# 0215Arthur/Pytorch_News_Recommender

Measured on AMD Instinct MI355X. Metric: users/sec (train step) NRMS MIND-small hist=50 cand=5, higher is better.
Workload: dtype f16 (MFMA inputs and saved activations; fp32 accumulate, softmax, loss, master weights and Adam); 1 GPU; configs[1] shapes: NRMS(nrms_v0) train step, 512 users/GPU, hist=50, cand=5, title_len=30, d=300, h=10, q=200, V=45800, dropout=0.2, Adam(lr=1e-3); users_per_gpu=512, global_batch=512, parallelism=dp1, precision=fp16, resident_batches=32

## Files before the change

### pytorch_news_recommender_amd/csrc/fused16_bwd.h

```cpp
#pragma once
#include "fused16.h"

namespace nrms {

constexpr int B16_RED_QKV = 3 * 10 * 32;
constexpr int B16_RED = B16_RED_QKV + 2 * F16_QP;
constexpr int B16_DQ = 96 * 10;

struct Bwd16Args {
    int n_seq, S, d, h, dk, q;
    int n_groups;
    const _Float16* x16;
    const int* pos;
    const int* n_rows;
    const int64_t* ids;
    const int* order;
    const int* order_cnt;
    int n_cls;
    const _Float16* btiles;
    const float* bqkv32;
    const _Float16* qv16;
    const _Float16* ctx16;
    const _Float16* t16;
    const float* w;
    const _Float16* dout16;
    _Float16* dz16;
    _Float16* dctx16;
    _Float16* dqkv16;
    float* red;
    Dropout drop;
    int v1;
    int dbg;
};

__device__ __forceinline__ f32x16 transpose32(const f32x16& x, const h8 (&idf)[2]) {
    f32x16 z = mfma32h(acc_frag(x, 0), idf[0], zero16());
    return mfma32h(acc_frag(x, 1), idf[1], z);
}

__device__ __forceinline__ float regsum(const f32x16& x) {
    float s0 = 0.f, s1 = 0.f, s2 = 0.f, s3 = 0.f;
#pragma unroll
    for (int g = 0; g < 4; ++g) { s0 += x[4 * g]; s1 += x[4 * g + 1]; s2 += x[4 * g + 2]; s3 += x[4 * g + 3]; }
    return (s0 + s1) + (s2 + s3);
}

__device__ __forceinline__ f32x16 transpose_frags(const h8& x0, const h8& x1, const h8 (&idf)[2]) {
    f32x16 z = mfma32h(x0, idf[0], zero16());
    return mfma32h(x1, idf[1], z);
}

constexpr int DX_BM = 256, DX_BK = 64, DX_THREADS = 512;
constexpr int DX_SLABS = B16_DQ / DX_BK;
constexpr int DX_A_BYTES = DX_BM * DX_BK * 2;
constexpr int DX_B_BYTES = DX_BK * F16_KP * 2;
constexpr int DX_SLOT = DX_A_BYTES + DX_B_BYTES;
static_assert(B16_DQ % DX_BK == 0 && F16_KP == 320, "15 slabs of 64; 10 column tiles of 32");
struct Dx16Args {
    int M;
    const int* m_dev;
    const _Float16* a16;
    const _Float16* xtiles;
    int lda, n_slabs;
    float* c;
    int ldc, d;
    const float* sc;
};


size_t bwd16_fused_lds(bool two_blocks);
int launch_bwd16_pool(const Bwd16Args& a, int n_wg, bool two_blocks, hipStream_t stream);
int launch_dx16(const Dx16Args& g, bool out16, hipStream_t stream);
int launch_dout16(long n_seq, int d, int h, int dk, float fixed_scale, float* sc, const float* dout, _Float16* dout16, hipStream_t stream);
int launch_tn16(int geom, const _Float16* A, int lda, int N, const _Float16* B, int ldb, int K, int M, const int* m_dev,
                float* partial, int splits, const int* nmap, const int* kmap, const float* nscale, int ldw, float* dW,
                hipStream_t stream, const char* name, float* dbias = nullptr, const int* blk_list = nullptr, const int* blk_cnt = nullptr,
                int blk_stride = 0);

}
```

### pytorch_news_recommender_amd/csrc/fused16_bwd.hip

```cpp
#include <stdlib.h>

#include "fused16_bwd.h"

namespace nrms {

template <int SB>
__global__ __launch_bounds__(F16_THREADS, SB == 1 ? 8 / F16_WAVES : 1) void fused_bwd16_pool_kernel(Bwd16Args a) {
    extern __shared__ __attribute__((aligned(16))) char smem[];
    float* red = reinterpret_cast<float*>(smem + 3 * F16_SLOT);
    float* stg_t = red + B16_RED;
    float* stg_h = stg_t + F16_WAVES * SB * 2 * F16_QT * 32;
    const int tid = threadIdx.x, lane = tid & 63;
    const int wave = __builtin_amdgcn_readfirstlane(tid >> 6);
    const int l32 = lane & 31, hh = lane >> 5;
    const int S = a.S;
    constexpr int DP = F16_DP, QP = F16_QP;

    for (int i = tid; i < B16_RED; i += F16_THREADS) red[i] = 0.f;

    h8 idf[2], sel[2];
#pragma unroll
    for (int s = 0; s < 2; ++s)
#pragma unroll
        for (int j = 0; j < 8; ++j) {
// ... 429 lines not shown
                            dk = mfma32h(acc_frag(q, 1), acc_frag(dsn, 1), dk);
                        }
                        const h8 dk0 = acc_frag(dk, 0), dk1 = acc_frag(dk, 1);
                        if (drow[jb] >= 0) {
                            *reinterpret_cast<h8*>(orow + 32) = dk0;
                            *reinterpret_cast<h8*>(orow + 32 + 16) = dk1;
                        }
                        sk += regsum(transpose_frags(dk0, dk1, idf));
                    }
                }
                sk += __shfl_xor(sk, 32, 64);
                if (hh == 0) srow[32] = sk;
                float sq = 0.f;
#pragma unroll
                for (int ib = 0; ib < SB; ++ib) {
                    f32x16 dq = zero16();
#pragma unroll
                    for (int jb = 0; jb < SB; ++jb) {
                        const f32x16 k = transpose_frags(kf[jb][0], kf[jb][1], idf);
                        dq = mfma32h(acc_frag(k, 0), sf[jb][ib][0], dq);
                        dq = mfma32h(acc_frag(k, 1), sf[jb][ib][1], dq);
                    }
                    const h8 dq0 = acc_frag(dq, 0), dq1 = acc_frag(dq, 1);
                    if (drow[ib] >= 0) {
                        _Float16* orow = a.dqkv16 + drow[ib] * (long)B16_DQ + head * 96 + 8 * hh;
                        *reinterpret_cast<h8*>(orow) = dq0;
                        *reinterpret_cast<h8*>(orow + 16) = dq1;
                    }
                    sq += regsum(transpose_frags(dq0, dq1, idf));
                }
                sq += __shfl_xor(sq, 32, 64);
                if (hh == 0) srow[0] = sq;
            }
            __syncthreads();
            if (tid < 96) {
                float sum = 0.f;
#pragma unroll
                for (int w = 0; w < F16_WAVES; ++w) sum += stg[(((head & 1) * F16_WAVES + w) * 3) * 32 + tid];
                red[3 * head * 32 + tid] += sum;
            }
            ++n;
        }
#pragma unroll
        for (int b = 0; b < SB; ++b) {
            if (drow[b] >= 0) {
                for (int head = a.h; head < 10; ++head) {
                    _Float16* orow = a.dqkv16 + drow[b] * (long)B16_DQ + head * 96 + 8 * hh;
#pragma unroll
                    for (int c = 0; c < 96; c += 16) *reinterpret_cast<h8*>(orow + c) = z8;
                }
            }
        }
        __syncthreads();
    }
    __syncthreads();
    float* out = a.red + (long)blockIdx.x * B16_RED;
    for (int i = tid; i < B16_RED; i += F16_THREADS) out[i] = red[i];
}

__device__ __forceinline__ float loss_scale_from_max(unsigned max_bits, float fixed) {
    if (fixed > 0.f) return fixed;
    const int e = (int)((max_bits >> 23) & 0xFF) - 127;
    if (max_bits == 0u || e == 128) return 1.0f;
    int k = 6 - e + (int)fmaxf(fixed, -24.f);
    k = k < -100 ? -100 : (k > 100 ? 100 : k);
    return __uint_as_float((unsigned)(k + 127) << 23);
}

__global__ __launch_bounds__(256) void absmax_kernel(long n, const float* x, unsigned* max_bits) {
    unsigned m = 0u;
    const long tid = (long)blockIdx.x * blockDim.x + threadIdx.x, nth = (long)gridDim.x * blockDim.x;
    if ((reinterpret_cast<uintptr_t>(x) & 15) == 0) {
        const f32x4* x4 = reinterpret_cast<const f32x4*>(x);
        const long n4 = n / 4;
        long i = tid;
        for (; i + 3 * nth < n4; i += 4 * nth) {
            f32x4 v[4];
#pragma unroll
            for (int u = 0; u < 4; ++u) v[u] = x4[i + u * nth];
#pragma unroll
            for (int u = 0; u < 4; ++u)
#pragma unroll
                for (int e = 0; e < 4; ++e) m = max(m, __float_as_uint(v[u][e]) & 0x7FFFFFFFu);
        }
        for (; i < n4; i += nth) {
            const f32x4 v = x4[i];
#pragma unroll
            for (int e = 0; e < 4; ++e) m = max(m, __float_as_uint(v[e]) & 0x7FFFFFFFu);
        }
        for (long i = (n & ~3L) + tid; i < n; i += nth) m = max(m, __float_as_uint(x[i]) & 0x7FFFFFFFu);
    } else {
        for (long i = tid; i < n; i += nth) m = max(m, __float_as_uint(x[i]) & 0x7FFFFFFFu);
    }
#pragma unroll
    for (int o = 32; o > 0; o >>= 1) m = max(m, (unsigned)__shfl_xor((int)m, o, 64));
    __shared__ unsigned wmax[4];
    if ((threadIdx.x & 63) == 0) wmax[threadIdx.x >> 6] = m;
    __syncthreads();
    if (threadIdx.x == 0) {
        m = max(max(wmax[0], wmax[1]), max(wmax[2], wmax[3]));
        if (m != 0u) atomicMax(max_bits, m);
    }
}

__device__ __forceinline__ void dout16_rows(long n_seq, int d, int h, int dk, float scale, float* sc, const float* dout, _Float16* dout16,
                                            int n_blocks) {
    if (blockIdx.x == 0 && threadIdx.x == 0) { sc[0] = scale; sc[1] = 1.0f / scale; }
    const long total = n_seq * F16_DP;
    for (long i = (long)blockIdx.x * blockDim.x + threadIdx.x; i < total; i += (long)n_blocks * blockDim.x) {
        const long r = i / F16_DP;
        const int p = (int)(i - r * F16_DP);
        const int b16 = p >> 4, t = p & 15, hh = t >> 3, jj = t & 7;
        const int fpad = 16 * b16 + 8 * (jj >> 2) + 4 * hh + (jj & 3);
        const int head = fpad >> 5, f = fpad & 31;
        float v = 0.f;
        if (head < h && f < dk) v = dout[r * d + head * dk + f] * scale;
        dout16[i] = (_Float16)v;
    }
}

__global__ __launch_bounds__(256) void dout16_kernel(long n_seq, int d, int h, int dk, float fixed_scale, const unsigned* max_bits,
                                                     float* sc, const float* dout, _Float16* dout16) {
    dout16_rows(n_seq, d, h, dk, loss_scale_from_max(*max_bits, fixed_scale), sc, dout, dout16, (int)gridDim.x);
}

struct Prep16bArgs {
    int d, h, dk, q;
    const float* w_qkv;
    const float* b_qkv;
    const float* w_add;
    const float* q_vec;
    float* bqkv32;
    _Float16* btiles;
    _Float16* xtiles;
    _Float16* qv16;
    unsigned* max_bits;
};

__global__ __launch_bounds__(256) void prep16b_kernel(Prep16bArgs a) {
    if (a.max_bits != nullptr && blockIdx.x == 0 && threadIdx.x == 0) *a.max_bits = 0u;
    const float qscale = 1.0f / sqrtf((float)a.dk);
    constexpr int KP = F16_KP;
    const long n1 = (long)4 * a.h * 32 * KP, n2 = (long)30 * 32 * KP, n3 = F16_QP, n4 = (long)3 * a.h * 32;
    for (long i = (long)blockIdx.x * blockDim.x + threadIdx.x; i < n1 + n2 + n3 + n4; i += (long)gridDim.x * blockDim.x) {
        if (i < n1) {
            const int c = (int)(i % KP);
            const long r = i / KP;
            const int f = (int)(r & 31), tile = (int)(r >> 5);
            float v = 0.f;
            if (tile < a.h) {
                const int head = tile;
                if (f < a.dk && c < a.q) v = a.w_add[(long)c * a.d + head * a.dk + f];
            } else {
                const int t3 = tile - a.h, head = t3 / 3, which = t3 - 3 * head;
                if (f < a.dk && c < a.d)
                    v = a.w_qkv[((long)which * a.d + head * a.dk + f) * a.d + c] * (which == 0 ? qscale : 1.0f);
                if (f < a.dk && c == a.d) v = a.b_qkv[which * a.d + head * a.dk + f] * (which == 0 ? qscale : 1.0f);
            }
            a.btiles[i] = (_Float16)v;
        } else if (i < n1 + n2) {
            const long j = i - n1;
            const int e = (int)(j & 7), l = (int)((j >> 3) & 31), hh2 = (int)((j >> 8) & 1);
            long r = j >> 9;
            const int t = (int)(r % 10); r /= 10;
            const int s4 = (int)(r & 3), slab = (int)(r >> 2);
            const int m = 64 * slab + 16 * s4 + 8 * hh2 + e;
            const int k = 32 * t + l;
            const int head = m / 96, rem = m - head * 96, which = rem >> 5, p = rem & 31;
            const int s = p >> 4, tt = p & 15, hh = tt >> 3, jj = tt & 7;
            const int f = 16 * s + 8 * (jj >> 2) + 4 * hh + (jj & 3);
            float v = 0.f;
            if (head < a.h && f < a.dk && k < a.d)
                v = a.w_qkv[((long)which * a.d + head * a.dk + f) * a.d + k] * (which == 0 ? qscale : 1.0f);
            a.xtiles[j] = (_Float16)v;
        } else if (i < n1 + n2 + n3) {
            const long j = i - n1 - n2;
            a.qv16[j] = (_Float16)(j < a.q ? a.q_vec[j] : 0.f);
        } else {
            const long j = i - n1 - n2 - n3;
            const int f = (int)(j & 31), tile = (int)(j >> 5), head = tile / 3, which = tile - 3 * head;
            a.bqkv32[j] = f < a.dk ? a.b_qkv[which * a.d + head * a.dk + f] * (which == 0 ? qscale : 1.0f) : 0.f;
        }
    }
}

template <bool OUT16>
__global__ __launch_bounds__(DX_THREADS, 2) void gemm16_dx_kernel(Dx16Args a) {
    extern __shared__ __attribute__((aligned(16))) char smem[];
    const int tid = threadIdx.x, lane = tid & 63;
    const int wave = __builtin_amdgcn_readfirstlane(tid >> 6);
    const int l32 = lane & 31, hh = lane >> 5;
    const int wm = wave >> 1, wn = wave & 1;
    const int M = a.m_dev != nullptr ? *a.m_dev : a.M;
    const int row0 = blockIdx.x * DX_BM;
    if (row0 >= M) return;
    const float inv_scale = a.sc[1];
    const char* asrc[4];
#pragma unroll
    for (int i = 0; i < 4; ++i) {
        const int r = 8 * (wave + 8 * i) + (lane >> 3);
        const int piece = (lane & 7) ^ ((r >> 1) & 7);
        asrc[i] = reinterpret_cast<const char*>(a.a16 + (long)min(row0 + r, M - 1) * a.lda) + piece * 16;
    }
    const char* bsrc = reinterpret_cast<const char*>(a.xtiles) + wave * 1024 + lane * 16;
    auto issue = [&](int slab, int slot) {
        char* la = smem + slot * DX_SLOT + wave * 1024;
#pragma unroll
        for (int i = 0; i < 4; ++i)
            __builtin_amdgcn_global_load_lds((const __attribute__((address_space(1))) void*)(asrc[i] + slab * (DX_BK * 2)),
                                             (__attribute__((address_space(3))) void*)(la + i * 8192), 16, 0, 0);
        char* lb = smem + slot * DX_SLOT + DX_A_BYTES + wave * 1024;
#pragma unroll
        for (int i = 0; i < 5; ++i)
            __builtin_amdgcn_global_load_lds((const __attribute__((address_space(1))) void*)(bsrc + (long)slab * DX_B_BYTES + i * 8192),
                                             (__attribute__((address_space(3))) void*)(lb + i * 8192), 16, 0, 0);
    };
    int aoff[2][4];
#pragma unroll
    for (int i = 0; i < 2; ++i) {
        const int r = wm * 64 + 32 * i + l32;
#pragma unroll
        for (int s = 0; s < 4; ++s) aoff[i][s] = r * 128 + (((2 * s + hh) ^ ((r >> 1) & 7)) << 4);
    }
    const int boff = DX_A_BYTES + (wn * 5 * 64 + lane) * 16;

    f32x16 acc[2][5];
#pragma unroll
    for (int i = 0; i < 2; ++i)
#pragma unroll
        for (int j = 0; j < 5; ++j) acc[i][j] = zero16();
    issue(0, 0);
    __asm__ volatile("s_waitcnt vmcnt(0)\n\ts_barrier" ::: "memory");
#pragma unroll 1
    for (int slab = 0; slab < a.n_slabs; ++slab) {
        if (slab + 1 < a.n_slabs) issue(slab + 1, (slab + 1) & 1);
        const char* st = smem + (slab & 1) * DX_SLOT;
#pragma unroll
        for (int s = 0; s < 4; ++s) {
            const h8 a0 = *reinterpret_cast<const h8*>(st + aoff[0][s]);
            const h8 a1 = *reinterpret_cast<const h8*>(st + aoff[1][s]);
#pragma unroll
            for (int j = 0; j < 5; ++j) {
                const h8 b = *reinterpret_cast<const h8*>(st + boff + (s * 10 + j) * 1024);
                acc[0][j] = mfma32h(b, a0, acc[0][j]);
                acc[1][j] = mfma32h(b, a1, acc[1][j]);
            }
        }
        __asm__ volatile("s_waitcnt vmcnt(0) lgkmcnt(0)\n\ts_barrier" ::: "memory");
    }
#pragma unroll
    for (int i = 0; i < 2; ++i) {
        const int row = row0 + wm * 64 + 32 * i + l32;
        if (row >= M) continue;
        float* crow = a.c + (long)row * a.ldc;
        _Float16* crow16 = reinterpret_cast<_Float16*>(a.c) + (long)row * F16_KP;
#pragma unroll
        for (int j = 0; j < 5; ++j)
#pragma unroll
            for (int g = 0; g < 4; ++g) {
                const int k = (wn * 5 + j) * 32 + 8 * g + 4 * hh;
                if (OUT16) {
                    h4 v;
#pragma unroll
                    for (int e = 0; e < 4; ++e) v[e] = (_Float16)acc[i][j][4 * g + e];
                    *reinterpret_cast<h4*>(crow16 + k) = v;
                } else if (k < a.d) {
                    f32x4 v;
#pragma unroll
                    for (int e = 0; e < 4; ++e) v[e] = acc[i][j][4 * g + e] * inv_scale;
                    *reinterpret_cast<f32x4*>(crow + k) = v;
                }
            }
    }
}

constexpr int T16_MC = 32, T16_THREADS = 512;
template <int WN, int NTN, int WK, int NTK>
struct Tn16Geom {
    static_assert(WN * WK * 64 == T16_THREADS, "eight waves");
    static constexpr int AW = 16 * WN * NTN, BW = 16 * WK * NTK;
    static constexpr int PA = AW + 16, PB = BW + 16;
    static_assert(((PA / 2) % 16) == 8 && ((PB / 2) % 16) == 8, "pitch = 8 * odd dwords (conflict-free transposed reads)");
    static constexpr int A_BYTES = T16_MC * PA * 2, B_BYTES = T16_MC * PB * 2;
    static constexpr int STAGE = A_BYTES + B_BYTES;
    static constexpr int A_IT = (T16_MC * AW / 8 + T16_THREADS - 1) / T16_THREADS;
    static constexpr int B_IT = (T16_MC * BW / 8 + T16_THREADS - 1) / T16_THREADS;
};
typedef Tn16Geom<4, 5, 2, 5> Tn16Qkv;
typedef Tn16Geom<2, 7, 4, 5> Tn16Add;

struct Tn16Args {
    int M;
    const int* m_dev;
    const _Float16* A; int lda, N;
    const _Float16* B; int ldb, K;
    float* partial;
    int splits, n_blk, k_blk;
    const int* blk_list; const int* blk_cnt; int blk_stride;
};

typedef short s16x4 __attribute__((ext_vector_type(4)));
typedef short s16x8 __attribute__((ext_vector_type(8)));

__device__ __forceinline__ h8 tr16_frag(const char* plane, int pitch_b, int col0, int lane) {
    const int l16 = lane & 15, kq = lane >> 4;
    const int q = l16 >> 2, p = l16 & 3;
    const char* a0 = plane + (4 * kq + q) * pitch_b + (col0 + 4 * p) * 2;
    const s16x4 lo4 = __builtin_amdgcn_ds_read_tr16_b64_v4i16((s16x4 __attribute__((address_space(3)))*)(a0));
    const s16x4 hi4 = __builtin_amdgcn_ds_read_tr16_b64_v4i16((s16x4 __attribute__((address_space(3)))*)(a0 + 16 * pitch_b));
    s16x8 r;
#pragma unroll
    for (int i = 0; i < 4; ++i) { r[i] = lo4[i]; r[4 + i] = hi4[i]; }
    return __builtin_bit_cast(h8, r);
}

template <bool FL, int WN, int NTN, int WK, int NTK>
__global__ __launch_bounds__(T16_THREADS, 2) void gemm16_tn_kernel(Tn16Args a) {
    typedef Tn16Geom<WN, NTN, WK, NTK> G;
    constexpr int T16_AW = G::AW, T16_BW = G::BW, T16_PA = G::PA, T16_PB = G::PB, T16_A_BYTES = G::A_BYTES;
    constexpr int T16_STAGE = G::STAGE, T16_A_IT = G::A_IT, T16_B_IT = G::B_IT, T16_NTN = NTN, T16_NTK = NTK;
    extern __shared__ __attribute__((aligned(16))) char smem[];
    const int tid = threadIdx.x, lane = tid & 63;
    const int wave = __builtin_amdgcn_readfirstlane(tid >> 6);
    const int wn = wave / WK, wk = wave % WK;
    const int out_blocks = a.n_blk * a.k_blk;
    const int per_xcd = gridDim.x >> 3;
    const int idx = (gridDim.x & 7) == 0 ? (blockIdx.x & 7) * per_xcd + (blockIdx.x >> 3) : blockIdx.x;
    const int blk = idx % out_blocks, split = idx / out_blocks;
    const int bn = blk % a.n_blk, bk = blk / a.n_blk;
    const int ncol0 = bn * T16_AW, kcol0 = bk * T16_BW;
    const int n_list0 = (FL && a.blk_list != nullptr) ? a.blk_cnt[0] : 0;
    const int M = (FL && a.blk_list != nullptr) ? 32 * (n_list0 + a.blk_cnt[2]) : (a.m_dev != nullptr ? *a.m_dev : a.M);
    const int rps = (((M + a.splits - 1) / a.splits) + T16_MC - 1) / T16_MC * T16_MC;
    const int m_begin = split * rps, m_end = min(M, m_begin + rps);

    struct Regs { h8 a[T16_A_IT], b[T16_B_IT]; };
    auto slot_rc = [&](int sl, int width, int& r, int& c) {
        if (FL) { r = (sl >> 1) & 31; c = (sl >> 6) * 16 + (sl & 1) * 8; if (c >= width) r = T16_MC; }
        else { r = sl / (width / 8); c = (sl % (width / 8)) * 8; }
    };
    auto load_stage = [&](Regs& R, int m0) {
        long blk = min(m0, max(m_end - 1, 0)) >> 5;
        if (FL && a.blk_list != nullptr && M > 0) blk = blk < n_list0 ? a.blk_list[blk] : a.blk_list[2 * (long)a.blk_stride + blk - n_list0];
#pragma unroll
        for (int i = 0; i < T16_A_IT; ++i) {
            int r, c;
            slot_rc(tid + T16_THREADS * i, T16_AW, r, c);
            r = min(r, T16_MC - 1);
            const int cc = min(ncol0 + c, a.N - 8);
            if (FL) R.a[i] = *reinterpret_cast<const h8*>(a.A + (blk * (a.lda >> 4) + (cc >> 4)) * 512 + r * 16 + (cc & 8));
            else R.a[i] = *reinterpret_cast<const h8*>(a.A + (long)min(m0 + r, max(m_end - 1, 0)) * a.lda + cc);
        }
#pragma unroll
        for (int i = 0; i < T16_B_IT; ++i) {
            int r, c;
            slot_rc(tid + T16_THREADS * i, T16_BW, r, c);
            r = min(r, T16_MC - 1);
            const int cc = min(kcol0 + c, a.K - 8);
            if (FL) R.b[i] = *reinterpret_cast<const h8*>(a.B + (blk * (a.ldb >> 4) + (cc >> 4)) * 512 + r * 16 + (cc & 8));
            else R.b[i] = *reinterpret_cast<const h8*>(a.B + (long)min(m0 + r, max(m_end - 1, 0)) * a.ldb + cc);
        }
    };
    const h8 z8 = {0, 0, 0, 0, 0, 0, 0, 0};
    auto store_stage = [&](const Regs& R, int m0, char* st) {
#pragma unroll
        for (int i = 0; i < T16_A_IT; ++i) {
            int r, c;
            slot_rc(tid + T16_THREADS * i, T16_AW, r, c);
            if (r < T16_MC) {
                const bool ok = m0 + r < m_end && ncol0 + c < a.N;
                *reinterpret_cast<h8*>(st + (r * T16_PA + c) * 2) = ok ? R.a[i] : z8;
            }
        }
#pragma unroll
        for (int i = 0; i < T16_B_IT; ++i) {
            int r, c;
            slot_rc(tid + T16_THREADS * i, T16_BW, r, c);
            if (r < T16_MC) {
                const bool ok = m0 + r < m_end && kcol0 + c < a.K;
                *reinterpret_cast<h8*>(st + T16_A_BYTES + (r * T16_PB + c) * 2) = ok ? R.b[i] : z8;
            }
        }
    };
    f32x4 acc[T16_NTN][T16_NTK];
#pragma unroll
    for (int i = 0; i < T16_NTN; ++i)
#pragma unroll
        for (int j = 0; j < T16_NTK; ++j) acc[i][j] = f32x4{0.f, 0.f, 0.f, 0.f};
    auto compute = [&](const char* st) {
        h8 bf[T16_NTK];
#pragma unroll
        for (int j = 0; j < T16_NTK; ++j) bf[j] = tr16_frag(st + T16_A_BYTES, T16_PB * 2, (wk * T16_NTK + j) * 16, lane);
#pragma unroll
        for (int i = 0; i < T16_NTN; ++i) {
            const h8 af = tr16_frag(st, T16_PA * 2, (wn * T16_NTN + i) * 16, lane);
#pragma unroll
            for (int j = 0; j < T16_NTK; ++j) acc[i][j] = __builtin_amdgcn_mfma_f32_16x16x32_f16(af, bf[j], acc[i][j], 0, 0, 0);
        }
    };
    int n_stage = m_end > m_begin ? (m_end - m_begin + T16_MC - 1) / T16_MC : 0;
    if (n_stage > 0) {
        n_stage = (n_stage + 1) & ~1;
        Regs R0, R1;
        load_stage(R1, m_begin);
        store_stage(R1, m_begin, smem);
        load_stage(R0, m_begin + T16_MC);
        __syncthreads();
        auto body = [&](const Regs& Rs, Regs& Rl, int s) {
            load_stage(Rl, m_begin + (s + 2) * T16_MC);
            store_stage(Rs, m_begin + (s + 1) * T16_MC, smem + ((s + 1) & 1) * T16_STAGE);
            compute(smem + (s & 1) * T16_STAGE);
            __syncthreads();
        };
        for (int s = 0; s < n_stage; s += 2) {
            body(R0, R1, s);
            body(R1, R0, s + 1);
        }
    }
    float* slab = a.partial + (long)split * a.N * a.K;
    const int r16 = lane & 15, kq = lane >> 4;
#pragma unroll
    for (int i = 0; i < T16_NTN; ++i)
#pragma unroll
        for (int j = 0; j < T16_NTK; ++j)
#pragma unroll
            for (int reg = 0; reg < 4; ++reg) {
                const int nn = ncol0 + (wn * T16_NTN + i) * 16 + 4 * kq + reg;
                const int kk = kcol0 + (wk * T16_NTK + j) * 16 + r16;
                if (nn < a.N && kk < a.K) slab[(long)nn * a.K + kk] = acc[i][j][reg];
            }
}

__global__ void tn16_reduce_kernel(const float* partial, int splits, int N, int K, const int* nmap, const int* kmap,
                                   const float* nscale, int ldw, float* dW, float* dbias) {
    const long total = (long)N * K;
    for (long idx = (long)blockIdx.x * blockDim.x + threadIdx.x; idx < total; idx += (long)gridDim.x * blockDim.x) {
        const int n = (int)(idx / K), k = (int)(idx - (long)n * K);
        const int nd = nmap[n], kd = kmap[k];
        if (nd < 0 || kd == -1 || (kd < 0 && dbias == nullptr)) continue;
        const float* pp = partial + idx;
        float s[8] = {0.f, 0.f, 0.f, 0.f, 0.f, 0.f, 0.f, 0.f};
        int sp = 0;
        for (; sp + 8 <= splits; sp += 8) {
#pragma unroll
            for (int u = 0; u < 8; ++u) s[u] += pp[(long)(sp + u) * total];
        }
        for (; sp < splits; ++sp) s[0] += pp[(long)sp * total];
        const float tot = (((s[0] + s[1]) + (s[2] + s[3])) + ((s[4] + s[5]) + (s[6] + s[7]))) * nscale[n];
        if (kd >= 0) dW[(long)nd * ldw + kd] += tot;
        else dbias[nd] += tot;
    }
}

__global__ __launch_bounds__(1024) void red16_kernel(const float* red, int n_wg, int h, int dk, int d, int q, const float* sc,
                                                    float qscale, float* db_qkv, float* db_add, float* dq_vec) {
    const float inv_scale = sc[1];
    __shared__ float part[32][33];
    const int c = threadIdx.x & 31, rg = threadIdx.x >> 5;
    const int i = blockIdx.x * 32 + c;
    float s = 0.f;
    if (i < B16_RED) {
        float s0 = 0.f, s1 = 0.f, s2 = 0.f, s3 = 0.f;
        int g = rg;
        for (; g + 96 < n_wg; g += 128) {
            s0 += red[(long)g * B16_RED + i];
            s1 += red[(long)(g + 32) * B16_RED + i];
            s2 += red[(long)(g + 64) * B16_RED + i];
            s3 += red[(long)(g + 96) * B16_RED + i];
        }
        for (; g < n_wg; g += 32) s0 += red[(long)g * B16_RED + i];
        s = (s0 + s1) + (s2 + s3);
    }
    part[rg][c] = s;
    __syncthreads();
    if (rg != 0 || i >= B16_RED) return;
    s = 0.f;
#pragma unroll
    for (int r = 0; r < 32; ++r) s += part[r][c];
    s *= inv_scale;
    if (i < B16_RED_QKV) {
        const int tile = i >> 5, f = i & 31, head = tile / 3, which = tile - 3 * head;
        if (head < h && f < dk) db_qkv[which * d + head * dk + f] += s * (which == 0 ? qscale : 1.0f);
    } else if (i < B16_RED_QKV + F16_QP) {
        const int qq = i - B16_RED_QKV;
        if (qq < q) db_add[qq] += s;
    } else {
        const int qq = i - B16_RED_QKV - F16_QP;
        if (qq < q) dq_vec[qq] += s;
    }
}

struct Maps16 { int *nmap_qkv, *kmap_x, *nmap_add, *kmap_ctx; float *nscale_qkv, *nscale_add; };
__device__ __forceinline__ void maps16_entry(int i, int d, int h, int dk, int q, float inv_scale, float qscale, const Maps16& m) {
    int* const nmap_qkv = m.nmap_qkv; int* const kmap_x = m.kmap_x; int* const nmap_add = m.nmap_add; int* const kmap_ctx = m.kmap_ctx;
    float* const nscale_qkv = m.nscale_qkv; float* const nscale_add = m.nscale_add;
    if (i < B16_DQ) {
        const int head = i / 96, rem = i - head * 96, which = rem >> 5, p = rem & 31;
        const int s = p >> 4, t = p & 15, hh = t >> 3, jj = t & 7;
        const int f = 16 * s + 8 * (jj >> 2) + 4 * hh + (jj & 3);
        nmap_qkv[i] = (head < h && f < dk) ? which * d + head * dk + f : -1;
        nscale_qkv[i] = inv_scale * (which == 0 ? qscale : 1.0f);
    }
    if (i < F16_KP) kmap_x[i] = i < d ? i : -1;
    if (i < F16_QP) { nmap_add[i] = i < q ? i : -1; nscale_add[i] = inv_scale; }
    if (i < F16_DP) {
        const int b16 = i >> 4, t = i & 15, hh = t >> 3, jj = t & 7;
        const int fpad = 16 * b16 + 8 * (jj >> 2) + 4 * hh + (jj & 3);
        const int head = fpad >> 5, f = fpad & 31;
        kmap_ctx[i] = (head < h && f < dk) ? head * dk + f : -1;
    }
}

constexpr int MAPS16_BLOCKS = (B16_DQ + 255) / 256;
static_assert(B16_DQ >= F16_KP && B16_DQ >= F16_QP && B16_DQ >= F16_DP, "maps16_entry: one thread per entry of the longest map");
__global__ __launch_bounds__(256) void dout16_maps_kernel(long n_seq, int d, int h, int dk, int q, float fixed_scale, float qscale,
                                                          const unsigned* max_bits, float* sc, const float* dout, _Float16* dout16,
                                                          Maps16 m) {
    const float scale = loss_scale_from_max(*max_bits, fixed_scale);
    const int n_rows_blocks = (int)gridDim.x - MAPS16_BLOCKS;
    if ((int)blockIdx.x >= n_rows_blocks) {
        maps16_entry(((int)blockIdx.x - n_rows_blocks) * 256 + (int)threadIdx.x, d, h, dk, q, 1.0f / scale, qscale, m);
        return;
    }
    dout16_rows(n_seq, d, h, dk, scale, sc, dout, dout16, n_rows_blocks);
}

static size_t up256(size_t x) { return (x + 255) / 256 * 256; }


Fused16BwdLayout fused16_bwd_layout(long M, int n_seq) {
    Fused16BwdLayout L;
    const long Mp = (long)n_seq * (M > (long)n_seq * 32 ? 64 : 32);
    size_t off = 0;
    auto take = [&](size_t bytes) { size_t o = off; off = up256(off + bytes); return o; };
    L.n_wg = 512;
    L.btiles = take((size_t)40 * 32 * F16_KP * 2);
    L.xtiles = take((size_t)DX_SLABS * DX_B_BYTES);
    L.qv16 = take((size_t)F16_QP * 2);
    L.bqkv32 = take((size_t)30 * 32 * 4);
    L.dout16 = take((size_t)n_seq * F16_DP * 2);
    L.dz16 = take((size_t)Mp * F16_QP * 2);
    L.dctx16 = take((size_t)Mp * F16_DP * 2);
    L.dqkv16 = take((size_t)(M + 32) * B16_DQ * 2);
    L.red = take((size_t)2 * L.n_wg * B16_RED * 4);
    L.maps = take((size_t)(B16_DQ * 2 + F16_KP + F16_QP * 2 + F16_DP) * 4);
    L.scale = take(256);
    L.tn_splits_qkv = 40;
    L.tn_splits_add = 192;
    if (const char* e = getenv("NRMS_TN_SPLITS_QKV")) L.tn_splits_qkv = atoi(e);
    if (const char* e = getenv("NRMS_TN_SPLITS_ADD")) L.tn_splits_add = atoi(e);
    const size_t p1 = (size_t)L.tn_splits_qkv * B16_DQ * F16_KP * 4, p2 = (size_t)L.tn_splits_add * F16_QP * F16_DP * 4;
    L.partial = take(up256(p1) + p2);
    L.total = off;
    return L;
}

int launch_tn16(int geom, const _Float16* A, int lda, int N, const _Float16* B, int ldb, int K, int M, const int* m_dev,
                float* partial, int splits, const int* nmap, const int* kmap, const float* nscale, int ldw, float* dW,
                hipStream_t stream, const char* name, float* dbias, const int* blk_list, const int* blk_cnt, int blk_stride) {
    Tn16Args t{};
    t.M = M; t.m_dev = m_dev; t.A = A; t.lda = lda; t.N = N; t.B = B; t.ldb = ldb; t.K = K; t.partial = partial;
    t.blk_list = geom != 0 ? blk_list : nullptr; t.blk_cnt = blk_cnt; t.blk_stride = blk_stride;
    typedef void (*Kern)(Tn16Args);
    const Kern fn = geom == 1 ? (Kern)gemm16_tn_kernel<true, 2, 7, 4, 5> : geom == 2 ? (Kern)gemm16_tn_kernel<true, 4, 5, 2, 5>
                                                                                     : (Kern)gemm16_tn_kernel<false, 4, 5, 2, 5>;
    const int aw = geom == 1 ? Tn16Add::AW : Tn16Qkv::AW, bw = geom == 1 ? Tn16Add::BW : Tn16Qkv::BW;
    t.splits = splits; t.n_blk = cdiv(N, aw); t.k_blk = cdiv(K, bw);
    const size_t lds = 2 * (size_t)(geom == 1 ? Tn16Add::STAGE : Tn16Qkv::STAGE);
    const hipError_t e = hipFuncSetAttribute((const void*)fn, hipFuncAttributeMaxDynamicSharedMemorySize, (int)lds);
    if (e != hipSuccess) { set_error("%s: hipFuncSetAttribute: %s", name, hipGetErrorString(e)); return NRMS_ELAUNCH; }
    {
        TimingScope ts(name, stream);
        hipLaunchKernelGGL(fn, dim3(splits * t.n_blk * t.k_blk), dim3(T16_THREADS), lds, stream, t);
    }
    int rc = check_launch(name);
    if (rc) return rc;
    TimingScope ts("tn_reduce", stream);
    hipLaunchKernelGGL(tn16_reduce_kernel, dim3(cdiv((long)N * K, 256)), dim3(256), 0, stream, partial, splits, N, K, nmap, kmap,
                       nscale, ldw, dW, dbias);
    return check_launch("tn16_reduce");
}

size_t bwd16_fused_lds(bool two) {
    static_assert(F16_WAVES * 2 * F16_QT * 32 + 2 * F16_WAVES * 32 >= 2 * F16_WAVES * 3 * 32, "the attention kernel's staging fits the same size");
    return (size_t)3 * F16_SLOT + (size_t)B16_RED * 4 + (size_t)(F16_WAVES * (two ? 2 : 1) * 2 * F16_QT * 32 + 2 * F16_WAVES * 32) * 4;
}

int launch_bwd16_pool(const Bwd16Args& a, int n_wg, bool two, hipStream_t stream) {
    const size_t lds = bwd16_fused_lds(two);
    const void* fp = two ? (const void*)fused_bwd16_pool_kernel<2> : (const void*)fused_bwd16_pool_kernel<1>;
    const hipError_t e = hipFuncSetAttribute(fp, hipFuncAttributeMaxDynamicSharedMemorySize, (int)lds);
    if (e != hipSuccess) { set_error("fused_bwd16: hipFuncSetAttribute: %s", hipGetErrorString(e)); return NRMS_ELAUNCH; }
    TimingScope ts(two ? "fused64_bwd16_pool" : "fused_bwd16_pool", stream);
    if (two) hipLaunchKernelGGL(fused_bwd16_pool_kernel<2>, dim3(n_wg), dim3(F16_THREADS), lds, stream, a);
    else hipLaunchKernelGGL(fused_bwd16_pool_kernel<1>, dim3(n_wg), dim3(F16_THREADS), lds, stream, a);
    return check_launch("fused_bwd16_pool");
}

int launch_dx16(const Dx16Args& g, bool out16, hipStream_t stream) {
    if ((g.d & 3) != 0 || ((uintptr_t)g.c & 15) != 0) { set_error("gemm16_dx: dx must be 16-byte aligned, d %% 4 == 0"); return NRMS_EINVAL; }
    const size_t lds = (size_t)2 * DX_SLOT;
    const void* fn = out16 ? (const void*)gemm16_dx_kernel<true> : (const void*)gemm16_dx_kernel<false>;
    const hipError_t e = hipFuncSetAttribute(fn, hipFuncAttributeMaxDynamicSharedMemorySize, (int)lds);
    if (e != hipSuccess) { set_error("gemm16_dx: hipFuncSetAttribute: %s", hipGetErrorString(e)); return NRMS_ELAUNCH; }
    TimingScope ts("dx_bwd", stream);
    if (out16) hipLaunchKernelGGL(gemm16_dx_kernel<true>, dim3(cdiv(g.M, DX_BM)), dim3(DX_THREADS), lds, stream, g);
    else hipLaunchKernelGGL(gemm16_dx_kernel<false>, dim3(cdiv(g.M, DX_BM)), dim3(DX_THREADS), lds, stream, g);
    return check_launch("gemm16_dx");
}

int launch_dout16(long n_seq, int d, int h, int dk, float fixed_scale, float* sc, const float* dout, _Float16* dout16, hipStream_t stream) {
    unsigned* max_bits = (unsigned*)(sc + 2);
    if (hipMemsetAsync(max_bits, 0, sizeof(unsigned), stream) != hipSuccess) { set_error("fused_bwd16: memset failed"); return NRMS_ELAUNCH; }
    const long nd = n_seq * d;
    if (!(fixed_scale > 0.f))
        hipLaunchKernelGGL(absmax_kernel, dim3(nd > 512L * 1024 ? 512 : (int)cdiv(nd, 1024)), dim3(256), 0, stream, nd, dout, max_bits);
    hipLaunchKernelGGL(dout16_kernel, dim3(cdiv(n_seq * F16_DP, 256) > 4096 ? 4096 : cdiv(n_seq * F16_DP, 256)),
                       dim3(256), 0, stream, n_seq, d, h, dk, fixed_scale, max_bits, sc, dout, dout16);
    return check_launch("dout16");
}

static int launch_dout16_maps(long n_seq, int d, int h, int dk, int q, float fixed_scale, float qscale, float* sc, const float* dout,
                              _Float16* dout16, const Maps16& m, hipStream_t stream) {
    unsigned* max_bits = (unsigned*)(sc + 2);
    const long nd = n_seq * d;
    if (!(fixed_scale > 0.f))
        hipLaunchKernelGGL(absmax_kernel, dim3(nd > 512L * 1024 ? 512 : (int)cdiv(nd, 1024)), dim3(256), 0, stream, nd, dout, max_bits);
    const int row_blocks = cdiv(n_seq * F16_DP, 256) > 4096 ? 4096 : cdiv(n_seq * F16_DP, 256);
    hipLaunchKernelGGL(dout16_maps_kernel, dim3(row_blocks + MAPS16_BLOCKS), dim3(256), 0, stream, n_seq, d, h, dk, q, fixed_scale,
                       qscale, max_bits, sc, dout, dout16, m);
    return check_launch("dout16");
}

int launch_fused_bwd16(const Fused16Bwd& f, hipStream_t stream) {
    if (f.n_seq <= 0) return NRMS_OK;
    const long M = (long)f.n_seq * f.S;
    const Fused16BwdLayout L = fused16_bwd_layout(M, f.n_seq);
    char* base = (char*)f.workspace;
    const int dk = f.d / f.h;
    const float qscale = 1.0f / sqrtf((float)dk);
    _Float16* btiles = (_Float16*)(base + L.btiles);
    _Float16* xtiles = (_Float16*)(base + L.xtiles);
    _Float16* qv16 = (_Float16*)(base + L.qv16);
    float* bqkv32 = (float*)(base + L.bqkv32);
    _Float16* dout16 = (_Float16*)(base + L.dout16);
    _Float16* dz16 = (_Float16*)(base + L.dz16);
    _Float16* dctx16 = (_Float16*)(base + L.dctx16);
    _Float16* dqkv16 = (_Float16*)(base + L.dqkv16);
    float* red = (float*)(base + L.red);
    int* nmap_qkv = (int*)(base + L.maps);
    float* nscale_qkv = (float*)(nmap_qkv + B16_DQ);
    int* kmap_x = (int*)(nscale_qkv + B16_DQ);
    int* nmap_add = kmap_x + F16_KP;
    float* nscale_add = (float*)(nmap_add + F16_QP);
    int* kmap_ctx = (int*)(nscale_add + F16_QP);
    float* sc = (float*)(base + L.scale);
    if (f.sc_out != nullptr) *f.sc_out = sc;
    float* partial_qkv = (float*)(base + L.partial);
    float* partial_add = (float*)(base + L.partial + up256((size_t)L.tn_splits_qkv * B16_DQ * F16_KP * 4));
    { const int jr = fused_bwd16_join(stream, false); if (jr) return jr; }
    SideSet* ss = side_streams_for(stream);
    const bool side = ss != nullptr;
    hipStream_t s_add = side ? ss->s[0] : stream, s_qkv = side ? ss->s[1] : stream;
    SideJoinGuard join_guard(ss, stream);
    const int Mp = f.n_seq * 32 * (f.S > 32 ? 2 : 1);
    {
        Prep16bArgs p{};
        p.d = f.d; p.h = f.h; p.dk = dk; p.q = f.q; p.w_qkv = f.w_qkv; p.b_qkv = f.b_qkv; p.w_add = f.w_add; p.q_vec = f.q_vec;
        p.btiles = btiles; p.xtiles = xtiles; p.qv16 = qv16; p.bqkv32 = bqkv32;
        p.max_bits = (unsigned*)(sc + 2);
        TimingScope ts("prep16", stream);
        hipLaunchKernelGGL(prep16b_kernel, dim3(2048), dim3(256), 0, stream, p);
        int rc = check_launch("prep16b");
        if (rc) return rc;
        Maps16 mp;
        mp.nmap_qkv = nmap_qkv; mp.nscale_qkv = nscale_qkv; mp.kmap_x = kmap_x; mp.nmap_add = nmap_add; mp.nscale_add = nscale_add;
        mp.kmap_ctx = kmap_ctx;
        rc = launch_dout16_maps((long)f.n_seq, f.d, f.h, dk, f.q, f.loss_scale, qscale, sc, f.dout, dout16, mp, stream);
        if (rc) return rc;
    }
    Bwd16Args a{};
    a.n_seq = f.n_seq; a.S = f.S; a.d = f.d; a.h = f.h; a.dk = dk; a.q = f.q;
    const bool lists = f.order != nullptr && f.S <= 32;
    a.n_groups = cdiv(f.n_seq, F16_WAVES) + (lists ? 2 : 0);
    a.n_cls = lists ? 3 : 2;
    a.x16 = (const _Float16*)f.x16; a.pos = f.pos; a.n_rows = f.n_rows_dev; a.ids = f.ids;
    a.order = lists ? f.order : nullptr; a.order_cnt = lists ? f.order_cnt : nullptr;
    a.btiles = btiles; a.bqkv32 = bqkv32; a.qv16 = qv16;
    a.ctx16 = (const _Float16*)f.ctx16; a.t16 = (const _Float16*)f.t16; a.w = f.w; a.dout16 = dout16;
    a.dz16 = dz16; a.dctx16 = dctx16; a.dqkv16 = dqkv16; a.red = red; a.drop = f.drop;
    a.dbg = 0;
#ifdef NRMS_F16_EXPERIMENTS
    { const char* e = getenv("NRMS_F16_DBG"); a.dbg = e ? atoi(e) : 0; }
#endif
    const int n_wg = a.n_groups < L.n_wg ? a.n_groups : L.n_wg;
    {
        const bool two = f.S > 32;
        const size_t lds = bwd16_fused_lds(two);
        const void* fa = two ? (const void*)fused_bwd16_attn_kernel<2> : (const void*)fused_bwd16_attn_kernel<1>;
        const hipError_t e = hipFuncSetAttribute(fa, hipFuncAttributeMaxDynamicSharedMemorySize, (int)lds);
        if (e != hipSuccess) { set_error("fused_bwd16: hipFuncSetAttribute: %s", hipGetErrorString(e)); return NRMS_ELAUNCH; }
        {
            const int rcp = launch_bwd16_pool(a, n_wg, two, stream);
            if (rcp) return rcp;
        }
        if (side) {
            int rc = side_order(ss, 0, stream, s_add, "fused_bwd16");
            if (rc) return rc;
            rc = launch_tn16(1, dz16, F16_QP, F16_QP, (const _Float16*)f.ctx16, F16_DP, F16_DP, Mp, nullptr, partial_add,
                             L.tn_splits_add, nmap_add, kmap_ctx, nscale_add, f.d, f.dw_add, s_add, "dwadd_bwd");
            if (rc) return rc;
            if (hipEventRecord(ss->ev[2], s_add) != hipSuccess) { set_error("fused_bwd16: hipEventRecord failed"); return NRMS_ELAUNCH; }
        }
        Bwd16Args b = a;
        b.red = red + (long)n_wg * B16_RED;
        {
            TimingScope ts(two ? "fused64_bwd16_attn" : "fused_bwd16_attn", stream);
            if (two) hipLaunchKernelGGL(fused_bwd16_attn_kernel<2>, dim3(n_wg), dim3(F16_THREADS), lds, stream, b);
            else hipLaunchKernelGGL(fused_bwd16_attn_kernel<1>, dim3(n_wg), dim3(F16_THREADS), lds, stream, b);
        }
        int rc = check_launch("fused_bwd16");
        if (rc) return rc;
    }
    int rc = NRMS_OK;
    if (!side) {
        rc = launch_tn16(1, dz16, F16_QP, F16_QP, (const _Float16*)f.ctx16, F16_DP, F16_DP, Mp, nullptr, partial_add,
                         L.tn_splits_add, nmap_add, kmap_ctx, nscale_add, f.d, f.dw_add, stream, "dwadd_bwd");
        if (rc) return rc;
    }
    if (side) {
        rc = side_order(ss, 1, stream, s_qkv, "fused_bwd16");
        if (rc) return rc;
    }
    rc = launch_tn16(0, dqkv16, B16_DQ, B16_DQ, (const _Float16*)f.x16, F16_KP, F16_KP, (int)M, f.n_rows_dev, partial_qkv,
                     L.tn_splits_qkv, nmap_qkv, kmap_x, nscale_qkv, f.d, f.dw_qkv, s_qkv, "dwqkv_bwd");
    if (rc) return rc;
    if (side && hipEventRecord(ss->ev[3], s_qkv) != hipSuccess) { set_error("fused_bwd16: hipEventRecord failed"); return NRMS_ELAUNCH; }
    {
        Dx16Args g{};
        g.M = (int)M; g.m_dev = f.n_rows_dev; g.a16 = dqkv16; g.xtiles = xtiles; g.c = f.dx; g.ldc = f.d; g.d = f.d;
        g.sc = sc; g.lda = B16_DQ; g.n_slabs = DX_SLABS;
        rc = launch_dx16(g, f.dx_fp16, stream);
    }
    if (rc == NRMS_OK) {
        TimingScope ts("red16", stream);
        hipLaunchKernelGGL(red16_kernel, dim3(cdiv(B16_RED, 32)), dim3(1024), 0, stream, red, 2 * n_wg, f.h, dk, f.d, f.q, sc,
                           qscale, f.db_qkv, f.db_add, f.dq_vec);
        rc = check_launch("red16");
    }
    if (side && rc == NRMS_OK) {
        if (f.defer_join) ss->pending = true;
        else if (hipStreamWaitEvent(stream, ss->ev[2], 0) != hipSuccess || hipStreamWaitEvent(stream, ss->ev[3], 0) != hipSuccess) {
            set_error("fused_bwd16: hipStreamWaitEvent failed");
            return NRMS_ELAUNCH;
        } else if ((rc = side_join_user(ss, stream, "fused_bwd16")) != NRMS_OK) return rc;
        join_guard.disarm();
    }
    return rc;
}

int fused_bwd16_join(hipStream_t stream, bool user) {
    SideSet* ss = side_streams_for(stream);
    if (ss == nullptr) return NRMS_OK;
    if (ss->pending) {
        ss->pending = false;
        if (hipStreamWaitEvent(stream, ss->ev[2], 0) != hipSuccess || hipStreamWaitEvent(stream, ss->ev[3], 0) != hipSuccess) {
            set_error("fused_bwd16_join: hipStreamWaitEvent failed");
            return NRMS_ELAUNCH;
        }
    }
    return user ? side_join_user(ss, stream, "fused_bwd16_join") : NRMS_OK;
}

}
```

Measured before the change: 175,500 users/s.

## Use direct global-to-LDS DMA with triple buffering in dW_qkv TN GEMM

Adds a variant of the TN weight-gradient GEMM in which full M-chunks are loaded with global_load_lds_dwordx4, so global data goes straight into LDS without passing through registers. It uses three LDS slots and vmcnt-based waits so that two stages are in flight while the current one is computed. The ragged tail falls back to the old register-staged path. The variant is enabled only for the dW_qkv launch when the shape and alignment checks pass. It needs more LDS per block, which may lower occupancy, and it relies on inline asm that manipulates m0.

```diff
diff --git a/pytorch_news_recommender_amd/csrc/fused16_bwd.h b/pytorch_news_recommender_amd/csrc/fused16_bwd.h
--- a/pytorch_news_recommender_amd/csrc/fused16_bwd.h
+++ b/pytorch_news_recommender_amd/csrc/fused16_bwd.h
@@ -75,6 +75,7 @@
 int launch_tn16(int geom, const _Float16* A, int lda, int N, const _Float16* B, int ldb, int K, int M, const int* m_dev,
                 float* partial, int splits, const int* nmap, const int* kmap, const float* nscale, int ldw, float* dW,
                 hipStream_t stream, const char* name, float* dbias = nullptr, const int* blk_list = nullptr, const int* blk_cnt = nullptr,
-                int blk_stride = 0);
+                int blk_stride = 0,
+                bool lds_dma = false);
 
 }
diff --git a/pytorch_news_recommender_amd/csrc/fused16_bwd.hip b/pytorch_news_recommender_amd/csrc/fused16_bwd.hip
--- a/pytorch_news_recommender_amd/csrc/fused16_bwd.hip
+++ b/pytorch_news_recommender_amd/csrc/fused16_bwd.hip
@@ -755,6 +755,16 @@
 typedef short s16x4 __attribute__((ext_vector_type(4)));
 typedef short s16x8 __attribute__((ext_vector_type(8)));
 
+__device__ __forceinline__ void glds16(const char* gsrc, unsigned lds_dst) {
+    unsigned keep;
+    __asm__ volatile("s_mov_b32 %0, m0\n\ts_mov_b32 m0, %2\n\ts_nop 0\n\tglobal_load_lds_dwordx4 %1, off\n\ts_mov_b32 m0, %0"
+                     : "=&s"(keep) : "v"(gsrc), "s"(lds_dst) : "memory");
+}
+
+template <int N> __device__ __forceinline__ void glds_wait_barrier() {
+    __asm__ volatile("s_waitcnt vmcnt(%0) lgkmcnt(0)\n\ts_barrier" :: "n"(N) : "memory");
+}
+
 __device__ __forceinline__ h8 tr16_frag(const char* plane, int pitch_b, int col0, int lane) {
     const int l16 = lane & 15, kq = lane >> 4;
     const int q = l16 >> 2, p = l16 & 3;
@@ -767,7 +777,7 @@
     return __builtin_bit_cast(h8, r);
 }
 
-template <bool FL, int WN, int NTN, int WK, int NTK>
+template <bool FL, int WN, int NTN, int WK, int NTK, bool DMA = false>
 __global__ __launch_bounds__(T16_THREADS, 2) void gemm16_tn_kernel(Tn16Args a) {
     typedef Tn16Geom<WN, NTN, WK, NTK> G;
     constexpr int T16_AW = G::AW, T16_BW = G::BW, T16_PA = G::PA, T16_PB = G::PB, T16_A_BYTES = G::A_BYTES;
@@ -852,7 +862,58 @@
         }
     };
     int n_stage = m_end > m_begin ? (m_end - m_begin + T16_MC - 1) / T16_MC : 0;
-    if (n_stage > 0) {
+    if constexpr (DMA) {
+        static_assert(!FL, "row-major operands");
+        constexpr int NSLOT = 3, NI = T16_STAGE / 1024, IT = NI / 8;
+        static_assert(T16_STAGE % 8192 == 0 && T16_A_BYTES % 1024 == 0, "whole wave instructions per operand, the same number per wave");
+        const int n_full = m_end > m_begin ? (m_end - m_begin) / T16_MC : 0;
+        unsigned off[IT];
+#pragma unroll
+        for (int i = 0; i < IT; ++i) {
+            const int j = i * 8 + wave;
+            const bool is_a = j * 1024 < T16_A_BYTES;
+            const int ch = (is_a ? j : j - T16_A_BYTES / 1024) * 64 + lane;
+            const int cpr = (is_a ? T16_PA : T16_PB) / 8;
+            const int r = ch / cpr;
+            int c = (ch - r * cpr) * 8;
+            if (c >= (is_a ? T16_AW : T16_BW)) c = 0;
+            off[i] = (unsigned)((r * (is_a ? a.lda : a.ldb) + (is_a ? ncol0 : kcol0) + c) * 2);
+        }
+        const char* const base_a = reinterpret_cast<const char*>(a.A) + (long)m_begin * a.lda * 2;
+        const char* const base_b = reinterpret_cast<const char*>(a.B) + (long)m_begin * a.ldb * 2;
+        const unsigned lds0 = (unsigned)(unsigned long)((__attribute__((address_space(3))) char*)smem);
+        auto issue = [&](int t, int slot) {
+            const char* const sa = base_a + (long)t * (T16_MC * 2) * a.lda;
+            const char* const sb = base_b + (long)t * (T16_MC * 2) * a.ldb;
+#pragma unroll
+            for (int i = 0; i < IT; ++i) {
+                const int j = i * 8 + wave;
+                glds16((j * 1024 < T16_A_BYTES ? sa : sb) + off[i], __builtin_amdgcn_readfirstlane(lds0 + slot * T16_STAGE + j * 1024));
+            }
+        };
+#pragma unroll
+        for (int t = 0; t < NSLOT - 1; ++t)
+            if (t < n_full) issue(t, t);
+        auto step = [&](int t, int slot) {
+            if (t + 1 < n_full) glds_wait_barrier<IT>();
+            else glds_wait_barrier<0>();
+            if (t + NSLOT - 1 < n_full) issue(t + NSLOT - 1, (slot + NSLOT - 1) % NSLOT);
+            compute(smem + slot * T16_STAGE);
+        };
+        for (int t0 = 0; t0 < n_full; t0 += NSLOT) {
+#pragma unroll
+            for (int u = 0; u < NSLOT; ++u)
+                if (t0 + u < n_full) step(t0 + u, u);
+        }
+        for (int s = n_full; s < ((n_stage + 1) & ~1); ++s) {
+            __syncthreads();
+            Regs R;
+            load_stage(R, m_begin + s * T16_MC);
+            store_stage(R, m_begin + s * T16_MC, smem);
+            __syncthreads();
+            compute(smem);
+        }
+    } else if (n_stage > 0) {
         n_stage = (n_stage + 1) & ~1;
         Regs R0, R1;
         load_stage(R1, m_begin);
@@ -1010,16 +1071,22 @@
 
 int launch_tn16(int geom, const _Float16* A, int lda, int N, const _Float16* B, int ldb, int K, int M, const int* m_dev,
                 float* partial, int splits, const int* nmap, const int* kmap, const float* nscale, int ldw, float* dW,
-                hipStream_t stream, const char* name, float* dbias, const int* blk_list, const int* blk_cnt, int blk_stride) {
+                hipStream_t stream, const char* name, float* dbias, const int* blk_list, const int* blk_cnt, int blk_stride,
+                bool lds_dma) {
     Tn16Args t{};
     t.M = M; t.m_dev = m_dev; t.A = A; t.lda = lda; t.N = N; t.B = B; t.ldb = ldb; t.K = K; t.partial = partial;
     t.blk_list = geom != 0 ? blk_list : nullptr; t.blk_cnt = blk_cnt; t.blk_stride = blk_stride;
     typedef void (*Kern)(Tn16Args);
-    const Kern fn = geom == 1 ? (Kern)gemm16_tn_kernel<true, 2, 7, 4, 5> : geom == 2 ? (Kern)gemm16_tn_kernel<true, 4, 5, 2, 5>
-                                                                                     : (Kern)gemm16_tn_kernel<false, 4, 5, 2, 5>;
+    Kern fn = geom == 1 ? (Kern)gemm16_tn_kernel<true, 2, 7, 4, 5> : geom == 2 ? (Kern)gemm16_tn_kernel<true, 4, 5, 2, 5>
+                                                                               : (Kern)gemm16_tn_kernel<false, 4, 5, 2, 5>;
     const int aw = geom == 1 ? Tn16Add::AW : Tn16Qkv::AW, bw = geom == 1 ? Tn16Add::BW : Tn16Qkv::BW;
     t.splits = splits; t.n_blk = cdiv(N, aw); t.k_blk = cdiv(K, bw);
-    const size_t lds = 2 * (size_t)(geom == 1 ? Tn16Add::STAGE : Tn16Qkv::STAGE);
+    size_t lds = 2 * (size_t)(geom == 1 ? Tn16Add::STAGE : Tn16Qkv::STAGE);
+    if (lds_dma && geom == 0 && getenv("NRMS_TN16_STAGED") == nullptr && N % aw == 0 && K % bw == 0 && lda % 8 == 0 && ldb % 8 == 0 &&
+        ((uintptr_t)A & 15) == 0 && ((uintptr_t)B & 15) == 0) {
+        fn = (Kern)gemm16_tn_kernel<false, 4, 5, 2, 5, true>;
+        lds = 3 * (size_t)Tn16Qkv::STAGE;
+    }
     const hipError_t e = hipFuncSetAttribute((const void*)fn, hipFuncAttributeMaxDynamicSharedMemorySize, (int)lds);
     if (e != hipSuccess) { set_error("%s: hipFuncSetAttribute: %s", name, hipGetErrorString(e)); return NRMS_ELAUNCH; }
     {
@@ -1186,7 +1253,7 @@
         if (rc) return rc;
     }
     rc = launch_tn16(0, dqkv16, B16_DQ, B16_DQ, (const _Float16*)f.x16, F16_KP, F16_KP, (int)M, f.n_rows_dev, partial_qkv,
-                     L.tn_splits_qkv, nmap_qkv, kmap_x, nscale_qkv, f.d, f.dw_qkv, s_qkv, "dwqkv_bwd");
+                     L.tn_splits_qkv, nmap_qkv, kmap_x, nscale_qkv, f.d, f.dw_qkv, s_qkv, "dwqkv_bwd", nullptr, nullptr, nullptr, 0, true);
     if (rc) return rc;
     if (side && hipEventRecord(ss->ev[3], s_qkv) != hipSuccess) { set_error("fused_bwd16: hipEventRecord failed"); return NRMS_ELAUNCH; }
     {
```

After: 176,300 users/s (median of 5 runs). No clear change (+0.5%).
